# liruihui/Dis-PU

Measured on AMD Instinct MI355X. Metric: upsampled points/sec (256->1024, 4x), higher is better.
Workload: dtype f32; 1 GPU; BASELINE configs[1]: 32 patches x 256 points per GPU, generator forward 256->1024 (4x), fp32; patches_per_gpu=32, global_patches=32, weights=xavier-uniform seed 1234, zero bias, parallelism=patch-sharded x1

## Files before the change

### dis-pu_amd/csrc/edge.hip

```cpp
#include "common.h"
#include "knn_select.h"


namespace dispu {

typedef float f32x16 __attribute__((ext_vector_type(16)));

template <int CTRL>
__device__ __forceinline__ float edge_dpp(float identity, float v) {
    return __int_as_float(__builtin_amdgcn_update_dpp(__float_as_int(identity), __float_as_int(v), CTRL, 0xF, 0xF, false));
}
__device__ __forceinline__ float edge_row16_max(float v) {
    v = fmaxf(v, edge_dpp<0x121>(v, v));
    v = fmaxf(v, edge_dpp<0x122>(v, v));
    v = fmaxf(v, edge_dpp<0x124>(v, v));
    v = fmaxf(v, edge_dpp<0x128>(v, v));
    return v;
}

__device__ __forceinline__ void edge_fill_frag(float* frag, const float* __restrict__ W, int K, int tid, int nthreads) {
    const int nf4 = K * 24 / 4;
    for (int e = tid; e < nf4; e += nthreads) {
        const float4 v = *reinterpret_cast<const float4*>(W + e * 4);
        const int k = (e * 4) / 24, ch0 = (e * 4) - k * 24;
        const float vv[4] = {v.x, v.y, v.z, v.w};
#pragma unroll
        for (int u = 0; u < 4; ++u) {
            const int ch = ch0 + u, r = ch >> 1, hp = ch & 1;
            const int i = (r & 3) | (hp << 2) | ((r >> 2) << 3);
            frag[(k >> 1) * 64 + (k & 1) * 32 + i] = vv[u];
        }
    }
    for (int e = tid; e < K * 8; e += nthreads) {
        const int sh = e >> 3;
        frag[sh * 32 + 24 + (e & 7)] = 0.f;
    }
}

__device__ __forceinline__ void edge_scatter_f4(float* frag, int e, const float4 v) {
    const int k = (e * 4) / 24, ch0 = (e * 4) - k * 24;
    const float vv[4] = {v.x, v.y, v.z, v.w};
#pragma unroll
    for (int u = 0; u < 4; ++u) {
        const int ch = ch0 + u, r = ch >> 1, hp = ch & 1;
        const int i = (r & 3) | (hp << 2) | ((r >> 2) << 3);
        frag[(k >> 1) * 64 + (k & 1) * 32 + i] = vv[u];
    }
}

constexpr int EK_NP = 64 * 4 + 4;
constexpr int EK_SCRATCH = 128 + 4;
constexpr int EK_KLD = 20;
constexpr int EK_MAXQ = 32;
template <int C, bool LDSF, bool PRE = false, bool KNN = false>
__global__ __launch_bounds__(LDSF ? 512 : 256) void edge_dense_conv_mfma_kernel(int npoints, int n_per_cloud, const float* __restrict__ F,
                                                                    long ldf, const int* __restrict__ idx, int ldi, int ioff,
                                                                    const float* __restrict__ W0, const float* __restrict__ b0,
                                                                    const float* __restrict__ W1, const float* __restrict__ b1,
                                                                    const float* __restrict__ W2, const float* __restrict__ b2,
                                                                    float* __restrict__ Y, long ldy, int* __restrict__ idx_out, int ksel,
                                                                    const float* __restrict__ Wp, const float* __restrict__ bp, int k_old,
                                                                    float* __restrict__ Pout, long ldp, const float* __restrict__ xyz,
                                                                    const float* __restrict__ Wl, const float* __restrict__ bl,
                                                                    float* __restrict__ Lout, long ldl) {
    constexpr int G = 24, H = C / 2, K0 = 2 * C, K1 = G + C, K2 = 2 * G + C;
    constexpr int S0 = K0 / 2, S1 = K1 / 2, S2 = K2 / 2;
    extern __shared__ __attribute__((aligned(16))) float edge_lds[];
#ifdef EDGE_STAMPS
    const unsigned long long e_k0 = __builtin_readcyclecounter();
#endif
    float* frag = edge_lds;
    float* stage = frag + (S0 + S1 + S2) * 64;
    constexpr int OWS = 3 * G + C + (KNN ? 4 : 0);
    float* fl = stage + (KNN ? EK_MAXQ : (LDSF ? 8 : 4) * 2) * OWS;
    static_assert(!PRE || LDSF, "the per-point prefix reads the LDS copy of the cloud");
    static_assert(!KNN || PRE, "the fused neighbour search is built on the LDS-resident, prefixed variant");
    const bool vec_store = ((ldy & 3) == 0) && ((((uintptr_t)Y) & 15) == 0);
    constexpr int FLD = C + 4;
    float* f0 = frag;
    float* f1 = frag + S0 * 64;
    float* f2 = f1 + S1 * 64;
    constexpr int NWAVE = LDSF ? 8 : 4;
    if constexpr (!LDSF) {
        edge_fill_frag(f0, W0, K0, threadIdx.x, 64 * NWAVE);
        edge_fill_frag(f1, W1, K1, threadIdx.x, 64 * NWAVE);
        edge_fill_frag(f2, W2, K2, threadIdx.x, 64 * NWAVE);
    }
    int cloud0 = 0, g_lo = 0, g_hi = (npoints + 1) / 2, gstep0 = gridDim.x * 4, gfirst = blockIdx.x * 4, per_wg = 0;
    if constexpr (LDSF) {
        const int parts = gridDim.y;
        const int cloud = blockIdx.x, part = blockIdx.y;
        cloud0 = cloud * n_per_cloud;
        const int gpc = n_per_cloud / 2;
        const int per = (gpc + parts - 1) / parts;
        per_wg = per;
        g_lo = cloud * gpc + part * per;
        g_hi = min(cloud * gpc + gpc, g_lo + per);
        gstep0 = NWAVE;
        gfirst = g_lo;
        constexpr int NT = 64 * NWAVE, N0 = K0 * 6, N1 = K1 * 6, N2 = K2 * 6, WB = (N0 + N1 + N2 + NT - 1) / NT, CB = 8;
        float4 wv[WB], cv[CB];
#pragma unroll
        for (int u = 0; u < WB; ++u) {
            const int e = min((int)threadIdx.x + u * NT, N0 + N1 + N2 - 1);
            const float* src = (e < N0) ? W0 + e * 4 : (e < N0 + N1) ? W1 + (e - N0) * 4 : W2 + (e - N0 - N1) * 4;
            wv[u] = *reinterpret_cast<const float4*>(src);
        }
        const int ctotal = n_per_cloud * (C / 4);
        const bool layer0 = KNN && C == 24 && xyz != nullptr;
        if (layer0) {
#pragma unroll
            for (int u = 0; u < CB; ++u) {
                const int e = (int)threadIdx.x + u * NT;
                if (u * NT < ctotal) {
                    const int ec = min(e, ctotal - 1);
                    const int p = ec / (C / 4), q = ec - p * (C / 4);
                    const float* xr = xyz + (size_t)(cloud0 + p) * 3;
                    float4 acc = make_float4(0.f, 0.f, 0.f, 0.f);
#pragma unroll
                    for (int k = 0; k < 3; ++k) {
                        const float x = xr[k];
                        const float4 w = *reinterpret_cast<const float4*>(Wl + k * 24 + q * 4);
                        acc.x = __builtin_fmaf(x, w.x, acc.x); acc.y = __builtin_fmaf(x, w.y, acc.y);
                        acc.z = __builtin_fmaf(x, w.z, acc.z); acc.w = __builtin_fmaf(x, w.w, acc.w);
                    }
                    const float4 b = *reinterpret_cast<const float4*>(bl + q * 4);
                    acc.x = acc.x + b.x; acc.y = acc.y + b.y; acc.z = acc.z + b.z; acc.w = acc.w + b.w;
                    cv[u] = acc;
                    const int pl = p - (g_lo * 2 - cloud0);
                    if (e < ctotal && pl >= 0 && pl < (g_hi - g_lo) * 2)
                        *reinterpret_cast<float4*>(Lout + (size_t)(cloud0 + p) * ldl + q * 4) = acc;
                }
            }
        } else {
#pragma unroll
            for (int u = 0; u < CB; ++u) {
                const int e = min((int)threadIdx.x + u * NT, ctotal - 1);
                const int p = e / (C / 4), q = e - p * (C / 4);
                cv[u] = *reinterpret_cast<const float4*>(F + (size_t)(cloud0 + p) * ldf + q * 4);
            }
        }
#pragma unroll
        for (int u = 0; u < WB; ++u) {
            const int e = (int)threadIdx.x + u * NT;
            if (e < N0) edge_scatter_f4(f0, e, wv[u]);
            else if (e < N0 + N1) edge_scatter_f4(f1, e - N0, wv[u]);
            else if (e < N0 + N1 + N2) edge_scatter_f4(f2, e - N0 - N1, wv[u]);
        }
        for (int e = threadIdx.x; e < (K0 + K1 + K2) * 8; e += NT)
            frag[(e >> 3) * 32 + 24 + (e & 7)] = 0.f;
#pragma unroll
        for (int u = 0; u < CB; ++u) {
            const int e = (int)threadIdx.x + u * NT;
            const int p = e / (C / 4), q = e - p * (C / 4);
            if (e < ctotal) *reinterpret_cast<float4*>(fl + p * FLD + q * 4) = cv[u];
        }
        if (!layer0)
            for (int e = threadIdx.x + CB * NT; e < ctotal; e += NT) {
                const int p = e / (C / 4), q = e - p * (C / 4);
                *reinterpret_cast<float4*>(fl + p * FLD + q * 4) = *reinterpret_cast<const float4*>(F + (size_t)(cloud0 + p) * ldf + q * 4);
            }
    }
    __syncthreads();
#ifdef EDGE_STAMPS
    const unsigned long long e_ka = __builtin_readcyclecounter();
    unsigned long long e_kb = e_ka, e_kc = e_ka;
#endif
    const int lane = threadIdx.x & 63, wave = threadIdx.x >> 6;
    const int row = lane & 31, h = lane >> 5;
    float* pre = fl + n_per_cloud * FLD;
    float* norms = pre + per_wg * 2 * 24;
    uint32_t* dmat = reinterpret_cast<uint32_t*>(norms + ((n_per_cloud + 3) & ~3));
    uint64_t* kscr = reinterpret_cast<uint64_t*>(dmat + EK_MAXQ * EK_NP);
    int* nbr = reinterpret_cast<int*>(kscr + NWAVE * EK_SCRATCH);
    const int n = n_per_cloud, p_base = g_lo * 2 - cloud0, ngl = g_hi - g_lo, nq = ngl * 2;
    typedef float ek_f32x4 __attribute__((ext_vector_type(4)));
    ek_f32x4 d00 = {0.f, 0.f, 0.f, 0.f}, d01 = d00, d10 = d00, d11 = d00;
    const int i16 = lane & 15, q4 = lane >> 4;
    const int ntile = (n + 15) >> 4;
    if constexpr (KNN) {
        for (int p = threadIdx.x; p < n; p += 64 * NWAVE) {
            const float* fr = fl + p * FLD;
            float r = 0.f;
#pragma unroll
            for (int c4 = 0; c4 < C / 4; ++c4) {
                const float4 v = *reinterpret_cast<const float4*>(fr + c4 * 4);
                r = __builtin_fmaf(v.x, v.x, r); r = __builtin_fmaf(v.y, v.y, r);
                r = __builtin_fmaf(v.z, v.z, r); r = __builtin_fmaf(v.w, v.w, r);
            }
            norms[p] = r;
        }
        if (wave < ntile) {
            const float* q0row = fl + min(p_base + i16, n - 1) * FLD + q4;
            const float* q1row = fl + min(p_base + 16 + i16, n - 1) * FLD + q4;
            const float* c0p = fl + min(wave * 16 + i16, n - 1) * FLD + q4;
            const float* c1p = fl + min((wave + NWAVE) * 16 + i16, n - 1) * FLD + q4;
#pragma unroll
            for (int c4 = 0; c4 < C / 4; ++c4) {
                const float a0 = q0row[c4 * 4], a1 = q1row[c4 * 4], b0v = c0p[c4 * 4], b1v = c1p[c4 * 4];
                d00 = __builtin_amdgcn_mfma_f32_16x16x4f32(a0, b0v, d00, 0, 0, 0);
                d01 = __builtin_amdgcn_mfma_f32_16x16x4f32(a0, b1v, d01, 0, 0, 0);
                d10 = __builtin_amdgcn_mfma_f32_16x16x4f32(a1, b0v, d10, 0, 0, 0);
                d11 = __builtin_amdgcn_mfma_f32_16x16x4f32(a1, b1v, d11, 0, 0, 0);
            }
        }
    }
    if constexpr (PRE) {
        const int npts_wg = nq;
        const int tw = KNN ? NWAVE - 1 - wave : wave;
        for (int t = tw; t * 32 < npts_wg; t += NWAVE) {
            const int pl = min(t * 32 + row, npts_wg - 1);
            const float* fr = fl + (p_base + pl) * FLD;
            f32x16 acc;
#pragma unroll
            for (int r = 0; r < 16; ++r) acc[r] = 0.f;
#pragma unroll
            for (int sq = 0; sq < C / 4; ++sq) {
                const float4 a = *reinterpret_cast<const float4*>(fr + sq * 4);
                acc = __builtin_amdgcn_mfma_f32_32x32x2f32(f0[(2 * sq) * 64 + lane], h ? a.y : a.x, acc, 0, 0, 0);
                acc = __builtin_amdgcn_mfma_f32_32x32x2f32(f0[(2 * sq + 1) * 64 + lane], h ? a.w : a.z, acc, 0, 0, 0);
            }
            if (t * 32 + row < npts_wg) {
                float* pp = pre + ((t * 32 + row) * 2 + h) * 12;
#pragma unroll
                for (int q = 0; q < 3; ++q)
                    *reinterpret_cast<float4*>(pp + q * 4) = make_float4(acc[4 * q], acc[4 * q + 1], acc[4 * q + 2], acc[4 * q + 3]);
            }
        }
        __syncthreads();
    }
#ifdef EDGE_STAMPS
    e_kb = __builtin_readcyclecounter();
#endif
    if constexpr (KNN) {
        if (wave < ntile) {
            const int cand0 = wave * 16 + i16, cand1 = cand0 + NWAVE * 16;
            const float rp0 = norms[min(cand0, n - 1)], rp1 = norms[min(cand1, n - 1)];
#pragma unroll
            for (int r = 0; r < 4; ++r) {
                const float rq0 = norms[min(p_base + 4 * q4 + r, n - 1)], rq1 = norms[min(p_base + 16 + 4 * q4 + r, n - 1)];
                uint32_t* m0 = dmat + (4 * q4 + r) * EK_NP;
                uint32_t* m1 = m0 + 16 * EK_NP;
                if (cand0 < n) {
                    m0[cand0] = f32_to_ordered(((rq0 - 2.0f * d00[r]) + rp0) + 0.0f);
                    if (nq > 16) m1[cand0] = f32_to_ordered(((rq1 - 2.0f * d10[r]) + rp0) + 0.0f);
                }
                if (cand1 < n) {
                    m0[cand1] = f32_to_ordered(((rq0 - 2.0f * d01[r]) + rp1) + 0.0f);
                    if (nq > 16) m1[cand1] = f32_to_ordered(((rq1 - 2.0f * d11[r]) + rp1) + 0.0f);
                }
            }
        }
        __syncthreads();
#ifdef EDGE_STAMPS
        e_kc = __builtin_readcyclecounter();
#endif
    }
    auto knn_select = [&](int gl) {
        if constexpr (KNN) {
            const int qa = 2 * gl, qb = qa + 1;
            uint32_t oda[4], odb[4];
            int cp[4];
#pragma unroll
            for (int r = 0; r < 4; ++r) {
                const int p = lane + 64 * r;
                cp[r] = p;
                oda[r] = (p < n) ? dmat[qa * EK_NP + p] : 0xFFFFFFFFu;
                odb[r] = (p < n) ? dmat[qb * EK_NP + p] : 0xFFFFFFFFu;
            }
            uint64_t* buf = kscr + (size_t)wave * EK_SCRATCH;
            int* outa = nbr + qa * EK_KLD;
            int* outb = nbr + qb * EK_KLD;
            const auto w2f = [](uint32_t w) { return ordered_to_f32(w); };
            const bool done_a = prefilter_rank<4, true>(oda, cp, buf, lane, ksel, 0xFFFFFFFEu, outa, nullptr, w2f);
            const bool done_b = prefilter_rank<4, true>(odb, cp, buf, lane, ksel, 0xFFFFFFFEu, outb, nullptr, w2f);
            if (!(done_a && done_b)) {
                uint64_t ka[4], kb[4];
#pragma unroll
                for (int r = 0; r < 4; ++r) {
                    ka[r] = (cp[r] < n) ? (((uint64_t)oda[r] << 32) | (uint32_t)cp[r]) : KEY_MAX;
                    kb[r] = (cp[r] < n) ? (((uint64_t)odb[r] << 32) | (uint32_t)cp[r]) : KEY_MAX;
                }
                sort_keys<4>(ka);
                sort_keys<4>(kb);
                uint64_t resa, resb;
                select_k2<4>(ka, kb, lane, ksel, resa, resb);
                if (lane < ksel) {
                    if (!done_a) outa[lane] = (int)(uint32_t)resa;
                    if (!done_b) outb[lane] = (int)(uint32_t)resb;
                }
            }
            if (idx_out != nullptr && lane < ksel) {
                int* o = idx_out + (size_t)(cloud0 + p_base + qa) * ksel;
                o[lane] = outa[lane];
                o[ksel + lane] = outb[lane];
            }
        }
    };
    if constexpr (KNN) {
        for (int gl = wave; gl < ngl; gl += NWAVE) knn_select(gl);
    }
#ifdef EDGE_STAMPS
    const unsigned long long e_k1 = __builtin_readcyclecounter();
#endif

    const int ngroups = LDSF ? g_hi : (npoints + 1) / 2;
    const int s_nb = row & 15;
    float4 ra[LDSF ? 1 : C / 4], rb[LDSF ? 1 : C / 4];
    int jl_next = 0;
    auto fetch = [&](int grp) {
        int p = grp * 2 + (row >> 4);
        if (p >= npoints) p = npoints - 1;
        if constexpr (KNN) {
            jl_next = nbr[(p - g_lo * 2) * EK_KLD + ioff + s_nb];
        } else if constexpr (LDSF) {
            jl_next = idx[(size_t)p * ldi + ioff + s_nb];
        } else {
            const int j = (p / n_per_cloud) * n_per_cloud + idx[(size_t)p * ldi + ioff + s_nb];
#pragma unroll
            for (int q = 0; q < C / 4; ++q) {
                ra[q] = *reinterpret_cast<const float4*>(F + (size_t)p * ldf + q * 4);
                rb[q] = *reinterpret_cast<const float4*>(F + (size_t)j * ldf + q * 4);
            }
        }
    };
    const int grp0 = gfirst + wave, gstride = gstep0;
    if (grp0 < ngroups) fetch(grp0);
    constexpr int SKIP = PRE ? H : 0;
    constexpr int WD = 12, STOT = S0 + S1 + S2 - SKIP;
    static_assert(STOT % WD == 0, "fragment ring depth must divide the step count");
    const float* fragG = frag + SKIP * 64;
    float wq[WD];
#pragma unroll
    for (int i = 0; i < WD; ++i) wq[i] = fragG[i * 64 + lane];
#ifdef EDGE_STAMPS
    unsigned long long e_conv = 0, e_l0 = 0, e_l1 = 0, e_l2 = 0, e_epi = 0, e_n = 0;
#define ED_T(v) __builtin_amdgcn_sched_barrier(0); const unsigned long long v = __builtin_readcyclecounter(); __builtin_amdgcn_sched_barrier(0)
#else
#define ED_T(v)
#endif
    float tail_bias = 0.f;
    if constexpr (KNN) {
        if (Wp != nullptr) tail_bias = bp[min(wave >> 1, 2) * 16 + i16];
    }
    for (int grp = grp0; grp < ngroups; grp += gstride) {
        ED_T(t0);
        float fp[H], df[H];
        const float* fp_ = fl + (grp * 2 + (row >> 4) - cloud0) * FLD;
        const float* fj_ = fl + jl_next * FLD;
#pragma unroll
        for (int q = 0; q < C / 4; ++q) {
            const float4 a = LDSF ? *reinterpret_cast<const float4*>(fp_ + q * 4) : ra[q];
            const float4 b = LDSF ? *reinterpret_cast<const float4*>(fj_ + q * 4) : rb[q];
            const float a0 = h ? a.y : a.x, a1 = h ? a.w : a.z;
            const float b0v = h ? b.y : b.x, b1v = h ? b.w : b.z;
            fp[2 * q] = a0; fp[2 * q + 1] = a1;
            df[2 * q] = b0v - a0; df[2 * q + 1] = b1v - a1;
        }
        if (grp + gstride < ngroups) fetch(grp + gstride);
        f32x16 l0, l1, l2;
#pragma unroll
        for (int r = 0; r < 16; ++r) { l0[r] = 0.f; l1[r] = 0.f; l2[r] = 0.f; }
        if constexpr (PRE) {
            const float* pp = pre + (((grp - g_lo) * 2 + (row >> 4)) * 2 + h) * 12;
#pragma unroll
            for (int q = 0; q < 3; ++q) {
                const float4 v = *reinterpret_cast<const float4*>(pp + q * 4);
                l0[4 * q] = v.x; l0[4 * q + 1] = v.y; l0[4 * q + 2] = v.z; l0[4 * q + 3] = v.w;
            }
        }
        auto step = [&](int sg, float bv, f32x16& acc) {
            const float w = wq[sg % WD];
            wq[sg % WD] = fragG[((sg + WD) % STOT) * 64 + lane];
            acc = __builtin_amdgcn_mfma_f32_32x32x2f32(w, bv, acc, 0, 0, 0);
        };
        ED_T(t1);
#pragma unroll
        for (int s = SKIP; s < S0; ++s) {
            const float bv = (s < H) ? fp[s < H ? s : 0] : df[s < H ? 0 : s - H];
            step(s - SKIP, bv, l0);
        }
#pragma unroll
        for (int r = 0; r < 12; ++r) l0[r] = fmaxf(l0[r] + b0[2 * r + h], 0.f);
        ED_T(t2);
#pragma unroll
        for (int s = 0; s < S1; ++s) {
            const float bv = (s < 12) ? l0[s < 12 ? s : 0] : fp[s < 12 ? 0 : s - 12];
            step(S0 - SKIP + s, bv, l1);
        }
#pragma unroll
        for (int r = 0; r < 12; ++r) l1[r] = fmaxf(l1[r] + b1[2 * r + h], 0.f);
        ED_T(t3);
#pragma unroll
        for (int s = 0; s < S2; ++s) {
            const float bv = (s < 12) ? l1[s < 12 ? s : 0] : ((s < 24) ? l0[(s >= 12 && s < 24) ? s - 12 : 0] : fp[s >= 24 ? s - 24 : 0]);
            step(S0 + S1 - SKIP + s, bv, l2);
        }
        ED_T(t4);
        constexpr int OW = 3 * G + C;
        float* stg = stage + (KNN ? (grp - g_lo) : wave) * (2 * OWS);
        float* sp = stg + (row >> 4) * OWS;
        float k2 = 0.f, k1 = 0.f, k0 = 0.f;
#pragma unroll
        for (int r = 0; r < 12; ++r) {
            float m2 = l2[r] + b2[2 * r + h], m1 = l1[r], m0 = l0[r];
            asm("s_nop 1\n\t"
                "v_max_f32_dpp %0, %0, %0 row_ror:1 row_mask:0xf bank_mask:0xf\n\t"
                "v_max_f32_dpp %1, %1, %1 row_ror:1 row_mask:0xf bank_mask:0xf\n\t"
                "v_max_f32_dpp %2, %2, %2 row_ror:1 row_mask:0xf bank_mask:0xf\n\t"
                "v_max_f32_dpp %0, %0, %0 row_ror:2 row_mask:0xf bank_mask:0xf\n\t"
                "v_max_f32_dpp %1, %1, %1 row_ror:2 row_mask:0xf bank_mask:0xf\n\t"
                "v_max_f32_dpp %2, %2, %2 row_ror:2 row_mask:0xf bank_mask:0xf\n\t"
                "v_max_f32_dpp %0, %0, %0 row_ror:4 row_mask:0xf bank_mask:0xf\n\t"
                "v_max_f32_dpp %1, %1, %1 row_ror:4 row_mask:0xf bank_mask:0xf\n\t"
                "v_max_f32_dpp %2, %2, %2 row_ror:4 row_mask:0xf bank_mask:0xf\n\t"
                "v_max_f32_dpp %0, %0, %0 row_ror:8 row_mask:0xf bank_mask:0xf\n\t"
                "v_max_f32_dpp %1, %1, %1 row_ror:8 row_mask:0xf bank_mask:0xf\n\t"
                "v_max_f32_dpp %2, %2, %2 row_ror:8 row_mask:0xf bank_mask:0xf"
                : "+v"(m2), "+v"(m1), "+v"(m0));
            k2 = (s_nb == r) ? m2 : k2; k1 = (s_nb == r) ? m1 : k1; k0 = (s_nb == r) ? m0 : k0;
        }
        if (s_nb < 12) { sp[2 * s_nb + h] = k2; sp[G + 2 * s_nb + h] = k1; sp[2 * G + 2 * s_nb + h] = k0; }
        {
            float fa = 0.f, fb = 0.f;
#pragma unroll
            for (int t = 0; t < H; ++t) {
                if (t < 16) fa = (s_nb == t) ? fp[t] : fa;
                else fb = (s_nb == t - 16) ? fp[t] : fb;
            }
            if (s_nb < (H < 16 ? H : 16)) sp[3 * G + 2 * s_nb + h] = fa;
            if (H > 16 && s_nb < H - 16) sp[3 * G + 2 * (s_nb + 16) + h] = fb;
        }
        const int p_first = grp * 2;
        if (vec_store) {
            if (lane < 2 * (OW / 4)) {
                const int pt = lane / (OW / 4), q4 = lane - pt * (OW / 4);
                if (p_first + pt < npoints)
                    *reinterpret_cast<float4*>(Y + (size_t)(p_first + pt) * ldy + q4 * 4) = *reinterpret_cast<const float4*>(stg + pt * OWS + q4 * 4);
            }
        } else {
            for (int e = lane; e < 2 * OW; e += 64) {
                const int pt = e / OW, q = e - pt * OW;
                if (p_first + pt < npoints) Y[(size_t)(p_first + pt) * ldy + q] = stg[pt * OWS + q];
            }
        }
#ifdef EDGE_STAMPS
        { ED_T(t5); e_conv += t1 - t0; e_l0 += t2 - t1; e_l1 += t3 - t2; e_l2 += t4 - t3; e_epi += t5 - t4; ++e_n; }
#endif
    }
#ifdef EDGE_STAMPS
    const unsigned long long e_p0 = __builtin_readcyclecounter();
    unsigned long long e_p1 = e_p0, e_p2 = e_p0, e_p3 = e_p0;
#endif
    if constexpr (KNN) {
        if (Wp != nullptr) {
            constexpr int OW = 3 * G + C, NT = 64 * NWAVE;
            const int K = OW + k_old, xld = k_old + 4;
            float* wl = fl;
            float* xl = frag;
            __syncthreads();
#ifdef EDGE_STAMPS
            e_p1 = __builtin_readcyclecounter();
#endif
            const int wtot = K * 12, xq = k_old >> 2, xtot = nq * xq;
            constexpr int TB_W = 9, TB_X = 4;
            float4 wv[TB_W], xv[TB_X];
#pragma unroll
            for (int u = 0; u < TB_W; ++u) wv[u] = *reinterpret_cast<const float4*>(Wp + (size_t)min((int)threadIdx.x + u * NT, wtot - 1) * 4);
#pragma unroll
            for (int u = 0; u < TB_X; ++u) {
                const int e = min((int)threadIdx.x + u * NT, max(xtot - 1, 0));
                const int pl = xq ? e / xq : 0, c4 = e - pl * xq;
                xv[u] = xtot ? *reinterpret_cast<const float4*>(Y + (size_t)(g_lo * 2 + pl) * ldy + OW + c4 * 4) : make_float4(0.f, 0.f, 0.f, 0.f);
            }
#pragma unroll
            for (int u = 0; u < TB_W; ++u) {
                const int e = (int)threadIdx.x + u * NT;
                if (e < wtot) *reinterpret_cast<float4*>(wl + e * 4) = wv[u];
            }
#pragma unroll
            for (int u = 0; u < TB_X; ++u) {
                const int e = (int)threadIdx.x + u * NT;
                const int pl = xq ? e / xq : 0, c4 = e - pl * xq;
                if (e < xtot) *reinterpret_cast<float4*>(xl + pl * xld + c4 * 4) = xv[u];
            }
            for (int e = threadIdx.x + TB_W * NT; e < wtot; e += NT)
                *reinterpret_cast<float4*>(wl + e * 4) = *reinterpret_cast<const float4*>(Wp + (size_t)e * 4);
            for (int e = threadIdx.x + TB_X * NT; e < xtot; e += NT) {
                const int pl = e / xq, c4 = e - pl * xq;
                *reinterpret_cast<float4*>(xl + pl * xld + c4 * 4) = *reinterpret_cast<const float4*>(Y + (size_t)(g_lo * 2 + pl) * ldy + OW + c4 * 4);
            }
            __syncthreads();
#ifdef EDGE_STAMPS
            e_p2 = __builtin_readcyclecounter();
#endif
            const int pt = wave & 1, ct = wave >> 1;
            if (ct < 3 && pt * 16 < nq) {
                const int pl = min(pt * 16 + i16, nq - 1);
                const float* xn = stage + pl * OWS + q4;
                const float* xo = xl + pl * xld + q4;
                const float* wp = wl + q4 * 48 + ct * 16 + i16;
                ek_f32x4 acc = {0.f, 0.f, 0.f, 0.f};
                const int nround = K / 24;
                float av[6], bv[6], an[6], bn[6];
                auto rd_load = [&](int rd, float (&a)[6], float (&b)[6]) {
                    rd = min(rd, nround - 1);
                    const float* xa = (rd < OW / 24) ? xn + rd * 24 : xo + (rd - OW / 24) * 24;
                    const float* wb = wp + rd * 24 * 48;
#pragma unroll
                    for (int u = 0; u < 6; ++u) { a[u] = xa[u * 4]; b[u] = wb[u * 4 * 48]; }
                };
                rd_load(0, av, bv);
                for (int rd = 0; rd < nround; rd += 2) {
                    rd_load(rd + 1, an, bn);
#pragma unroll
                    for (int u = 0; u < 6; ++u) acc = __builtin_amdgcn_mfma_f32_16x16x4f32(av[u], bv[u], acc, 0, 0, 0);
                    if (rd + 1 < nround) {
                        rd_load(rd + 2, av, bv);
#pragma unroll
                        for (int u = 0; u < 6; ++u) acc = __builtin_amdgcn_mfma_f32_16x16x4f32(an[u], bn[u], acc, 0, 0, 0);
                    }
                }
#ifdef EDGE_STAMPS
                __builtin_amdgcn_sched_barrier(0); e_p3 = __builtin_readcyclecounter(); __builtin_amdgcn_sched_barrier(0);
#endif
                const float bb = tail_bias;
#pragma unroll
                for (int r = 0; r < 4; ++r) {
                    const int pr = pt * 16 + 4 * q4 + r;
                    if (pr < nq) Pout[(size_t)(g_lo * 2 + pr) * ldp + ct * 16 + i16] = fmaxf(acc[r] + bb, 0.f);
                }
            }
        }
    }
#ifdef EDGE_STAMPS
    if (blockIdx.x == 3 && blockIdx.y == 0 && lane == 0) {
        unsigned long long* st = reinterpret_cast<unsigned long long*>(Y + (size_t)npoints * ldy) + wave * 16;
        st[11] = e_p1 - e_p0; st[12] = e_p2 - e_p1; st[13] = __builtin_readcyclecounter() - e_p2; st[14] = e_p3 - e_p2;
        st[0] = e_conv; st[1] = e_l0; st[2] = e_l1; st[3] = e_l2; st[4] = e_epi; st[5] = e_n; st[6] = e_ka - e_k0; st[7] = e_kb - e_ka;
        st[8] = e_kc - e_kb; st[9] = e_k1 - e_kc; st[10] = __builtin_readcyclecounter() - e_k0;
    }
#endif
}

}

using namespace dispu;

DISPU_EXPORT int dispu_edge_dense_conv(int npoints, int n_per_cloud, int C, const float* F, long ldf, const int* idx, int ldi,
                                       int ioff, const float* W0, const float* b0, const float* W1, const float* b1,
                                       const float* W2, const float* b2, float* Y, long ldy, void* stream) {
    if (npoints < 0 || n_per_cloud <= 0 || !(C == 24 || C == 48) || (ldf & 3) || (((uintptr_t)F) & 15)) return (int)hipErrorInvalidValue;
    if (npoints == 0) return 0;
    hipStream_t s = (hipStream_t)stream;
    const size_t frag_bytes = (size_t)((C == 24 ? 84 : 132) * 64 + 16 * (72 + C)) * sizeof(float);
    const size_t feat_bytes = (size_t)n_per_cloud * (C + 4) * sizeof(float);
    if (npoints % n_per_cloud == 0 && n_per_cloud % 2 == 0 && frag_bytes + feat_bytes <= 160 * 1024) {
        const int clouds = npoints / n_per_cloud;
        int parts = (256 + clouds - 1) / clouds;
        const int gpc = n_per_cloud / 2;
        if (parts > (gpc + 7) / 8) parts = (gpc + 7) / 8;
        if (parts < 1) parts = 1;
        const int per = (gpc + parts - 1) / parts;
        const size_t pre_bytes = (size_t)per * 2 * 24 * sizeof(float);
        const bool pre = frag_bytes + feat_bytes + pre_bytes <= 160 * 1024;
        const size_t bytes = frag_bytes + feat_bytes + (pre ? pre_bytes : 0);
        static DevOnce attr;      
        if (attr.needed()) {
            DISPU_TRY(hipFuncSetAttribute(reinterpret_cast<const void*>(edge_dense_conv_mfma_kernel<24, true>),
                                          hipFuncAttributeMaxDynamicSharedMemorySize, 160 * 1024));
            DISPU_TRY(hipFuncSetAttribute(reinterpret_cast<const void*>(edge_dense_conv_mfma_kernel<48, true>),
                                          hipFuncAttributeMaxDynamicSharedMemorySize, 160 * 1024));
            DISPU_TRY(hipFuncSetAttribute(reinterpret_cast<const void*>(edge_dense_conv_mfma_kernel<24, true, true>),
                                          hipFuncAttributeMaxDynamicSharedMemorySize, 160 * 1024));
            DISPU_TRY(hipFuncSetAttribute(reinterpret_cast<const void*>(edge_dense_conv_mfma_kernel<48, true, true>),
                                          hipFuncAttributeMaxDynamicSharedMemorySize, 160 * 1024));
            attr.done();
        }
#define EDGE_LAUNCH(C_, PRE_) hipLaunchKernelGGL((edge_dense_conv_mfma_kernel<C_, true, PRE_>), dim3(clouds, parts), dim3(512), bytes, s, npoints, \
                                                 n_per_cloud, F, ldf, idx, ldi, ioff, W0, b0, W1, b1, W2, b2, Y, ldy, nullptr, 0, nullptr, nullptr, 0, nullptr, 0, nullptr, nullptr, nullptr, nullptr, 0)
        if (C == 24) { if (pre) EDGE_LAUNCH(24, true); else EDGE_LAUNCH(24, false); }
        else { if (pre) EDGE_LAUNCH(48, true); else EDGE_LAUNCH(48, false); }
#undef EDGE_LAUNCH
        return (int)hipGetLastError();
    }
    int g = (npoints + 7) / 8;
    if (g > 256) g = 256;
    if (C == 24)
        hipLaunchKernelGGL((edge_dense_conv_mfma_kernel<24, false>), dim3(g), dim3(256), frag_bytes, s, npoints, n_per_cloud, F, ldf, idx, ldi, ioff, W0, b0, W1, b1, W2, b2, Y, ldy, nullptr, 0, nullptr, nullptr, 0, nullptr, 0, nullptr, nullptr, nullptr, nullptr, 0);
    else
        hipLaunchKernelGGL((edge_dense_conv_mfma_kernel<48, false>), dim3(g), dim3(256), frag_bytes, s, npoints, n_per_cloud, F, ldf, idx, ldi, ioff, W0, b0, W1, b1, W2, b2, Y, ldy, nullptr, 0, nullptr, nullptr, 0, nullptr, 0, nullptr, nullptr, nullptr, nullptr, 0);
    return (int)hipGetLastError();
}

DISPU_EXPORT int dispu_stem_block(int npoints, int n_per_cloud, int C, const float* F, long ldf, int ksel, int ioff, const float* W0,
                                  const float* b0, const float* W1, const float* b1, const float* W2, const float* b2, float* Y, long ldy,
                                  int* idx_out, const float* Wp, const float* bp, int k_old, float* P, long ldp, const float* xyz,
                                  const float* Wl, const float* bl, float* Lout, long ldl, void* stream) {
    if (xyz != nullptr && (C != 24 || Wl == nullptr || bl == nullptr || Lout == nullptr || (ldl & 3) || (((uintptr_t)Lout) & 15) ||
                           (((uintptr_t)Wl) & 15) || (((uintptr_t)bl) & 15) || n_per_cloud * 6 > 8 * 512))
        return (int)hipErrorInvalidValue;
    if (xyz == nullptr && F == nullptr) return (int)hipErrorInvalidValue;
    if (Wp != nullptr && (bp == nullptr || P == nullptr || k_old < 0 || k_old % 24 != 0 || ldp < 48)) return (int)hipErrorInvalidValue;
    if (npoints < 0 || n_per_cloud <= 0 || !(C == 24 || C == 48) || (ldf & 3) || (((uintptr_t)F) & 15)) return (int)hipErrorInvalidValue;
    if (n_per_cloud > 256 || (n_per_cloud & 1) || npoints % n_per_cloud != 0 || ioff < 0 || ksel != ioff + 16 || ksel > EK_KLD ||
        ksel > n_per_cloud)
        return (int)hipErrorInvalidValue;
    if (npoints == 0) return 0;
    hipStream_t s = (hipStream_t)stream;
    const int clouds = npoints / n_per_cloud, gpc = n_per_cloud / 2;
    int parts = (256 + clouds - 1) / clouds;
    if (parts > (gpc + 7) / 8) parts = (gpc + 7) / 8;
    if (parts < (gpc + EK_MAXQ / 2 - 1) / (EK_MAXQ / 2)) parts = (gpc + EK_MAXQ / 2 - 1) / (EK_MAXQ / 2);
    const int per = (gpc + parts - 1) / parts;
    const float* Wp_fused = Wp;
    if (Wp != nullptr) {
        const long wcap = (long)n_per_cloud * (C + 4) + per * 48 + ((n_per_cloud + 3) & ~3) + EK_MAXQ * EK_NP, xcap = (C == 24 ? 84 : 132) * 64;
        if ((ldy & 3) || (((uintptr_t)Y) & 15) || (((uintptr_t)Wp) & 15)) return (int)hipErrorInvalidValue;
        if ((long)(72 + C + k_old) * 48 > wcap || (long)per * 2 * (k_old + 4) > xcap) Wp_fused = nullptr;
    }
    const size_t bytes = (size_t)((C == 24 ? 84 : 132) * 64 + EK_MAXQ * (72 + C + 4)) * sizeof(float) + (size_t)n_per_cloud * (C + 4) * sizeof(float) +
                         (size_t)per * 2 * 24 * sizeof(float) + (size_t)((n_per_cloud + 3) & ~3) * sizeof(float) +
                         (size_t)EK_MAXQ * EK_NP * sizeof(uint32_t) + (size_t)8 * EK_SCRATCH * sizeof(uint64_t) + (size_t)EK_MAXQ * EK_KLD * sizeof(int);
    static DevOnce attr;
    if (attr.needed()) {
        DISPU_TRY(hipFuncSetAttribute(reinterpret_cast<const void*>(edge_dense_conv_mfma_kernel<24, true, true, true>),
                                      hipFuncAttributeMaxDynamicSharedMemorySize, 160 * 1024));
        DISPU_TRY(hipFuncSetAttribute(reinterpret_cast<const void*>(edge_dense_conv_mfma_kernel<48, true, true, true>),
                                      hipFuncAttributeMaxDynamicSharedMemorySize, 160 * 1024));
        attr.done();
    }
    if (C == 24)
        hipLaunchKernelGGL((edge_dense_conv_mfma_kernel<24, true, true, true>), dim3(clouds, parts), dim3(512), bytes, s, npoints, n_per_cloud, F, ldf,
                           nullptr, 0, ioff, W0, b0, W1, b1, W2, b2, Y, ldy, idx_out, ksel, Wp_fused, bp, k_old, P, ldp, xyz, Wl, bl, Lout, ldl);
    else
        hipLaunchKernelGGL((edge_dense_conv_mfma_kernel<48, true, true, true>), dim3(clouds, parts), dim3(512), bytes, s, npoints, n_per_cloud, F, ldf,
                           nullptr, 0, ioff, W0, b0, W1, b1, W2, b2, Y, ldy, idx_out, ksel, Wp_fused, bp, k_old, P, ldp, xyz, Wl, bl, Lout, ldl);
    const int rc = (int)hipGetLastError();
    if (rc != 0 || Wp == Wp_fused) return rc;
    return dispu_linear(1, npoints, 72 + C + k_old, 48, Y, ldy, 0, Wp, 48, 0, 0, bp, 1, P, ldp, 0, nullptr, 0, 0, nullptr, 0, 0, stream);
}
```

Before: 36.04 million points/s.

## Prefetch tail weights before barrier and software-pipeline tail MFMA LDS reads

The tail projection stage now has half the workgroup issue the global loads of the projection weights and per-point features before the barrier, so their latency overlaps the wait instead of following it. The tail MFMA loop is rewritten with inline ds_read asm and explicit lgkmcnt waits, keeping a ring of six in-flight LDS reads per operand ahead of the matrix ops. The stamp instrumentation is also reorganised into a uniform accumulator macro. Hand-written waitcnt counts and inline asm carry a correctness risk if the compiler adds LDS traffic of its own, and the fixed loader tile sizes assume particular channel widths.

```diff
diff --git a/dis-pu_amd/csrc/edge.hip b/dis-pu_amd/csrc/edge.hip
--- a/dis-pu_amd/csrc/edge.hip
+++ b/dis-pu_amd/csrc/edge.hip
@@ -46,6 +46,24 @@
         const int i = (r & 3) | (hp << 2) | ((r >> 2) << 3);
         frag[(k >> 1) * 64 + (k & 1) * 32 + i] = vv[u];
     }
+}
+
+__device__ __forceinline__ unsigned edge_lds_addr(const float* p) {
+    return (unsigned)(size_t)(const __attribute__((address_space(3))) float*)p;
+}
+template <int OFF> __device__ __forceinline__ void edge_dsread(float& dst, unsigned addr) {
+    asm volatile("ds_read_b32 %0, %1 offset:%2" : "=v"(dst) : "v"(addr), "n"(OFF) : "memory");
+}
+template <int N> __device__ __forceinline__ void edge_lds_wait(float& a, float& b) {
+    asm volatile("s_waitcnt lgkmcnt(%2)" : "+v"(a), "+v"(b) : "n"(N) : "memory");
+}
+__device__ __forceinline__ float4 edge_unset4() {
+    float4 v;
+    asm volatile("" : "=v"(v.x), "=v"(v.y), "=v"(v.z), "=v"(v.w));
+    return v;
+}
+__device__ __forceinline__ void edge_lds_settle() {
+    asm volatile("s_waitcnt lgkmcnt(0)" ::: "memory");
 }
 
 constexpr int EK_NP = 64 * 4 + 4;
@@ -67,7 +85,17 @@
     constexpr int S0 = K0 / 2, S1 = K1 / 2, S2 = K2 / 2;
     extern __shared__ __attribute__((aligned(16))) float edge_lds[];
 #ifdef EDGE_STAMPS
+    enum { ES_STAGE, ES_BAR_STAGE, ES_PHASE2, ES_BAR_PRE, ES_COMBINE, ES_BAR_COMBINE, ES_SELECT, ES_RING, ES_GATHER, ES_L0, ES_L1, ES_L2, ES_EPI,
+           ES_TAIL_ISSUE, ES_TAIL_WAIT, ES_TAIL_STAGE, ES_BAR_TAIL, ES_TAIL_LOOP, ES_TAIL_STORE, ES_N };
+    unsigned long long e_acc[ES_N], e_n = 0;
+#pragma unroll
+    for (int i = 0; i < ES_N; ++i) e_acc[i] = 0;
     const unsigned long long e_k0 = __builtin_readcyclecounter();
+    unsigned long long e_last = e_k0;
+#define ES(i) do { __builtin_amdgcn_sched_barrier(0); const unsigned long long t_ = __builtin_readcyclecounter(); e_acc[i] += t_ - e_last; e_last = t_; \
+                   __builtin_amdgcn_sched_barrier(0); } while (0)
+#else
+#define ES(i) do { } while (0)
 #endif
     float* frag = edge_lds;
     float* stage = frag + (S0 + S1 + S2) * 64;
@@ -161,11 +189,9 @@
                 *reinterpret_cast<float4*>(fl + p * FLD + q * 4) = *reinterpret_cast<const float4*>(F + (size_t)(cloud0 + p) * ldf + q * 4);
             }
     }
+    ES(ES_STAGE);
     __syncthreads();
-#ifdef EDGE_STAMPS
-    const unsigned long long e_ka = __builtin_readcyclecounter();
-    unsigned long long e_kb = e_ka, e_kc = e_ka;
-#endif
+    ES(ES_BAR_STAGE);
     const int lane = threadIdx.x & 63, wave = threadIdx.x >> 6;
     const int row = lane & 31, h = lane >> 5;
     float* pre = fl + n_per_cloud * FLD;
@@ -227,11 +253,10 @@
                     *reinterpret_cast<float4*>(pp + q * 4) = make_float4(acc[4 * q], acc[4 * q + 1], acc[4 * q + 2], acc[4 * q + 3]);
             }
         }
+        ES(ES_PHASE2);
         __syncthreads();
-    }
-#ifdef EDGE_STAMPS
-    e_kb = __builtin_readcyclecounter();
-#endif
+        ES(ES_BAR_PRE);
+    }
     if constexpr (KNN) {
         if (wave < ntile) {
             const int cand0 = wave * 16 + i16, cand1 = cand0 + NWAVE * 16;
@@ -251,10 +276,9 @@
                 }
             }
         }
+        ES(ES_COMBINE);
         __syncthreads();
-#ifdef EDGE_STAMPS
-        e_kc = __builtin_readcyclecounter();
-#endif
+        ES(ES_BAR_COMBINE);
     }
     auto knn_select = [&](int gl) {
         if constexpr (KNN) {
@@ -300,9 +324,7 @@
     if constexpr (KNN) {
         for (int gl = wave; gl < ngl; gl += NWAVE) knn_select(gl);
     }
-#ifdef EDGE_STAMPS
-    const unsigned long long e_k1 = __builtin_readcyclecounter();
-#endif
+    ES(ES_SELECT);
 
     const int ngroups = LDSF ? g_hi : (npoints + 1) / 2;
     const int s_nb = row & 15;
@@ -333,18 +355,12 @@
     float wq[WD];
 #pragma unroll
     for (int i = 0; i < WD; ++i) wq[i] = fragG[i * 64 + lane];
-#ifdef EDGE_STAMPS
-    unsigned long long e_conv = 0, e_l0 = 0, e_l1 = 0, e_l2 = 0, e_epi = 0, e_n = 0;
-#define ED_T(v) __builtin_amdgcn_sched_barrier(0); const unsigned long long v = __builtin_readcyclecounter(); __builtin_amdgcn_sched_barrier(0)
-#else
-#define ED_T(v)
-#endif
     float tail_bias = 0.f;
     if constexpr (KNN) {
         if (Wp != nullptr) tail_bias = bp[min(wave >> 1, 2) * 16 + i16];
     }
     for (int grp = grp0; grp < ngroups; grp += gstride) {
-        ED_T(t0);
+        ES(ES_RING);
         float fp[H], df[H];
         const float* fp_ = fl + (grp * 2 + (row >> 4) - cloud0) * FLD;
         const float* fj_ = fl + jl_next * FLD;
@@ -374,7 +390,7 @@
             wq[sg % WD] = fragG[((sg + WD) % STOT) * 64 + lane];
             acc = __builtin_amdgcn_mfma_f32_32x32x2f32(w, bv, acc, 0, 0, 0);
         };
-        ED_T(t1);
+        ES(ES_GATHER);
 #pragma unroll
         for (int s = SKIP; s < S0; ++s) {
             const float bv = (s < H) ? fp[s < H ? s : 0] : df[s < H ? 0 : s - H];
@@ -382,7 +398,7 @@
         }
 #pragma unroll
         for (int r = 0; r < 12; ++r) l0[r] = fmaxf(l0[r] + b0[2 * r + h], 0.f);
-        ED_T(t2);
+        ES(ES_L0);
 #pragma unroll
         for (int s = 0; s < S1; ++s) {
             const float bv = (s < 12) ? l0[s < 12 ? s : 0] : fp[s < 12 ? 0 : s - 12];
@@ -390,13 +406,13 @@
         }
 #pragma unroll
         for (int r = 0; r < 12; ++r) l1[r] = fmaxf(l1[r] + b1[2 * r + h], 0.f);
-        ED_T(t3);
+        ES(ES_L1);
 #pragma unroll
         for (int s = 0; s < S2; ++s) {
             const float bv = (s < 12) ? l1[s < 12 ? s : 0] : ((s < 24) ? l0[(s >= 12 && s < 24) ? s - 12 : 0] : fp[s >= 24 ? s - 24 : 0]);
             step(S0 + S1 - SKIP + s, bv, l2);
         }
-        ED_T(t4);
+        ES(ES_L2);
         constexpr int OW = 3 * G + C;
         float* stg = stage + (KNN ? (grp - g_lo) : wave) * (2 * OWS);
         float* sp = stg + (row >> 4) * OWS;
@@ -444,86 +460,87 @@
                 if (p_first + pt < npoints) Y[(size_t)(p_first + pt) * ldy + q] = stg[pt * OWS + q];
             }
         }
+        ES(ES_EPI);
 #ifdef EDGE_STAMPS
-        { ED_T(t5); e_conv += t1 - t0; e_l0 += t2 - t1; e_l1 += t3 - t2; e_l2 += t4 - t3; e_epi += t5 - t4; ++e_n; }
+        ++e_n;
 #endif
     }
-#ifdef EDGE_STAMPS
-    const unsigned long long e_p0 = __builtin_readcyclecounter();
-    unsigned long long e_p1 = e_p0, e_p2 = e_p0, e_p3 = e_p0;
-#endif
+    ES(ES_RING);
     if constexpr (KNN) {
         if (Wp != nullptr) {
             constexpr int OW = 3 * G + C, NT = 64 * NWAVE;
             const int K = OW + k_old, xld = k_old + 4;
             float* wl = fl;
             float* xl = frag;
+            constexpr int NTL = 64 * (NWAVE / 2), TB_W = C == 24 ? 6 : 18, TB_X = C == 24 ? 1 : 8;
+            const int wtot = K * 12, xq = k_old >> 2;
+            const bool loader = threadIdx.x < NTL;
+            static_assert(NTL / 8 == EK_MAXQ, "eight loader threads per point of the workgroup");
+            const int xr = (int)threadIdx.x >> 3, xc = (int)threadIdx.x & 7;
+            float4 wv[TB_W], xv[TB_X];
+#pragma unroll
+            for (int u = 0; u < TB_W; ++u) wv[u] = edge_unset4();
+#pragma unroll
+            for (int u = 0; u < TB_X; ++u) xv[u] = edge_unset4();
+            if (loader) {
+#pragma unroll
+                for (int u = 0; u < TB_W; ++u)
+                    wv[u] = *reinterpret_cast<const float4*>(reinterpret_cast<const char*>(Wp) + (unsigned)min((int)threadIdx.x + u * NTL, wtot - 1) * 16u);
+                if (xq) {
+                    const char* yr = reinterpret_cast<const char*>(Y + (size_t)(g_lo * 2 + min(xr, nq - 1)) * ldy + OW);
+#pragma unroll
+                    for (int u = 0; u < TB_X; ++u) xv[u] = *reinterpret_cast<const float4*>(yr + (unsigned)min(xc + 8 * u, xq - 1) * 16u);
+                }
+            }
+            ES(ES_TAIL_ISSUE);
             __syncthreads();
-#ifdef EDGE_STAMPS
-            e_p1 = __builtin_readcyclecounter();
-#endif
-            const int wtot = K * 12, xq = k_old >> 2, xtot = nq * xq;
-            constexpr int TB_W = 9, TB_X = 4;
-            float4 wv[TB_W], xv[TB_X];
-#pragma unroll
-            for (int u = 0; u < TB_W; ++u) wv[u] = *reinterpret_cast<const float4*>(Wp + (size_t)min((int)threadIdx.x + u * NT, wtot - 1) * 4);
-#pragma unroll
-            for (int u = 0; u < TB_X; ++u) {
-                const int e = min((int)threadIdx.x + u * NT, max(xtot - 1, 0));
-                const int pl = xq ? e / xq : 0, c4 = e - pl * xq;
-                xv[u] = xtot ? *reinterpret_cast<const float4*>(Y + (size_t)(g_lo * 2 + pl) * ldy + OW + c4 * 4) : make_float4(0.f, 0.f, 0.f, 0.f);
-            }
-#pragma unroll
-            for (int u = 0; u < TB_W; ++u) {
-                const int e = (int)threadIdx.x + u * NT;
-                if (e < wtot) *reinterpret_cast<float4*>(wl + e * 4) = wv[u];
-            }
-#pragma unroll
-            for (int u = 0; u < TB_X; ++u) {
-                const int e = (int)threadIdx.x + u * NT;
-                const int pl = xq ? e / xq : 0, c4 = e - pl * xq;
-                if (e < xtot) *reinterpret_cast<float4*>(xl + pl * xld + c4 * 4) = xv[u];
-            }
-            for (int e = threadIdx.x + TB_W * NT; e < wtot; e += NT)
+            ES(ES_TAIL_WAIT);
+            if (loader) {
+#pragma unroll
+                for (int u = 0; u < TB_W; ++u) {
+                    const int e = (int)threadIdx.x + u * NTL;
+                    if (e < wtot) *reinterpret_cast<float4*>(wl + e * 4) = wv[u];
+                }
+#pragma unroll
+                for (int u = 0; u < TB_X; ++u)
+                    if (xr < nq && xc + 8 * u < xq) *reinterpret_cast<float4*>(xl + xr * xld + (xc + 8 * u) * 4) = xv[u];
+            }
+            for (int e = threadIdx.x + TB_W * NTL; e < wtot; e += NT)
                 *reinterpret_cast<float4*>(wl + e * 4) = *reinterpret_cast<const float4*>(Wp + (size_t)e * 4);
-            for (int e = threadIdx.x + TB_X * NT; e < xtot; e += NT) {
-                const int pl = e / xq, c4 = e - pl * xq;
+            const int xrem = xq - 8 * TB_X;
+            for (int e = threadIdx.x; e < nq * xrem; e += NT) {
+                const int pl = e / xrem, c4 = 8 * TB_X + e - pl * xrem;
                 *reinterpret_cast<float4*>(xl + pl * xld + c4 * 4) = *reinterpret_cast<const float4*>(Y + (size_t)(g_lo * 2 + pl) * ldy + OW + c4 * 4);
             }
+            ES(ES_TAIL_STAGE);
             __syncthreads();
-#ifdef EDGE_STAMPS
-            e_p2 = __builtin_readcyclecounter();
-#endif
+            ES(ES_BAR_TAIL);
             const int pt = wave & 1, ct = wave >> 1;
             if (ct < 3 && pt * 16 < nq) {
                 const int pl = min(pt * 16 + i16, nq - 1);
-                const float* xn = stage + pl * OWS + q4;
-                const float* xo = xl + pl * xld + q4;
-                const float* wp = wl + q4 * 48 + ct * 16 + i16;
                 ek_f32x4 acc = {0.f, 0.f, 0.f, 0.f};
                 const int nround = K / 24;
-                float av[6], bv[6], an[6], bn[6];
-                auto rd_load = [&](int rd, float (&a)[6], float (&b)[6]) {
-                    rd = min(rd, nround - 1);
-                    const float* xa = (rd < OW / 24) ? xn + rd * 24 : xo + (rd - OW / 24) * 24;
-                    const float* wb = wp + rd * 24 * 48;
-#pragma unroll
-                    for (int u = 0; u < 6; ++u) { a[u] = xa[u * 4]; b[u] = wb[u * 4 * 48]; }
-                };
-                rd_load(0, av, bv);
-                for (int rd = 0; rd < nround; rd += 2) {
-                    rd_load(rd + 1, an, bn);
-#pragma unroll
-                    for (int u = 0; u < 6; ++u) acc = __builtin_amdgcn_mfma_f32_16x16x4f32(av[u], bv[u], acc, 0, 0, 0);
-                    if (rd + 1 < nround) {
-                        rd_load(rd + 2, av, bv);
-#pragma unroll
-                        for (int u = 0; u < 6; ++u) acc = __builtin_amdgcn_mfma_f32_16x16x4f32(an[u], bn[u], acc, 0, 0, 0);
-                    }
-                }
-#ifdef EDGE_STAMPS
-                __builtin_amdgcn_sched_barrier(0); e_p3 = __builtin_readcyclecounter(); __builtin_amdgcn_sched_barrier(0);
-#endif
+                const unsigned xn = edge_lds_addr(stage + pl * OWS + q4), xo = edge_lds_addr(xl + pl * xld + q4);
+                unsigned wb = edge_lds_addr(wl + q4 * 48 + ct * 16 + i16);
+                float av[6], bv[6];
+                edge_lds_settle();
+#define EDGE_RING_READ(u, xa_) edge_dsread<16 * (u)>(av[u], xa_); edge_dsread<16 * 48 * (u)>(bv[u], wb)
+#define EDGE_RING_MFMA(u, n_) edge_lds_wait<n_>(av[u], bv[u]); acc = __builtin_amdgcn_mfma_f32_16x16x4f32(av[u], bv[u], acc, 0, 0, 0)
+                EDGE_RING_READ(0, xn); EDGE_RING_READ(1, xn); EDGE_RING_READ(2, xn); EDGE_RING_READ(3, xn); EDGE_RING_READ(4, xn); EDGE_RING_READ(5, xn);
+                for (int rd = 1; rd < nround; ++rd) {
+                    const unsigned xa = (rd < OW / 24) ? xn + rd * 96 : xo + (rd - OW / 24) * 96;
+                    wb += 24 * 48 * 4;
+                    EDGE_RING_MFMA(0, 10); EDGE_RING_READ(0, xa);
+                    EDGE_RING_MFMA(1, 10); EDGE_RING_READ(1, xa);
+                    EDGE_RING_MFMA(2, 10); EDGE_RING_READ(2, xa);
+                    EDGE_RING_MFMA(3, 10); EDGE_RING_READ(3, xa);
+                    EDGE_RING_MFMA(4, 10); EDGE_RING_READ(4, xa);
+                    EDGE_RING_MFMA(5, 10); EDGE_RING_READ(5, xa);
+                }
+                EDGE_RING_MFMA(0, 10); EDGE_RING_MFMA(1, 8); EDGE_RING_MFMA(2, 6); EDGE_RING_MFMA(3, 4); EDGE_RING_MFMA(4, 2); EDGE_RING_MFMA(5, 0);
+#undef EDGE_RING_READ
+#undef EDGE_RING_MFMA
+                ES(ES_TAIL_LOOP);
                 const float bb = tail_bias;
 #pragma unroll
                 for (int r = 0; r < 4; ++r) {
@@ -533,14 +550,16 @@
             }
         }
     }
+    ES(ES_TAIL_STORE);
 #ifdef EDGE_STAMPS
     if (blockIdx.x == 3 && blockIdx.y == 0 && lane == 0) {
-        unsigned long long* st = reinterpret_cast<unsigned long long*>(Y + (size_t)npoints * ldy) + wave * 16;
-        st[11] = e_p1 - e_p0; st[12] = e_p2 - e_p1; st[13] = __builtin_readcyclecounter() - e_p2; st[14] = e_p3 - e_p2;
-        st[0] = e_conv; st[1] = e_l0; st[2] = e_l1; st[3] = e_l2; st[4] = e_epi; st[5] = e_n; st[6] = e_ka - e_k0; st[7] = e_kb - e_ka;
-        st[8] = e_kc - e_kb; st[9] = e_k1 - e_kc; st[10] = __builtin_readcyclecounter() - e_k0;
+        unsigned long long* st = reinterpret_cast<unsigned long long*>(Y + (size_t)npoints * ldy) + wave * 32;
+#pragma unroll
+        for (int i = 0; i < ES_N; ++i) st[i] = e_acc[i];
+        st[ES_N] = e_n; st[ES_N + 1] = e_last - e_k0;
     }
 #endif
+#undef ES
 }
 
 }
```

After: 36.35 million points/s, median of 5. No clear change (+0.9%).
